# hwb0314/VI-ORB-SLAM-ICRA2018

Hardware: AMD Instinct MI355X
Metric: ORB extract+match frames/sec @640x480/1000 feat (higher is better)
Workload: dtype u8

## Files before the change

vi-orb-slam-icra2018_amd/csrc/k_pyramid.hip:

```cpp
#include "orbhip_internal.h"
#include "wave_ops.h"

#include <algorithm>

#define RZ_TW 128
typedef unsigned short us2 __attribute__((ext_vector_type(2)));
#define RZ_MAXCH 16
#define RZ_MAXROWS 44

template <int RZ_TH>
__global__ __launch_bounds__(256) void k_resize(const uint8_t *__restrict__ src, int sstride,
                                                unsigned long long sframe, uint8_t *__restrict__ dst,
                                                int dw, int dh, int dstride, unsigned long long dframe,
                                                const int2 *__restrict__ xtab,
                                                const int4 *__restrict__ ytab, const int4 *__restrict__ gtab, int sw, int sh,
                                                float winx, float winy, int xcdMap)
{
    __shared__ __align__(16) uint8_t s_src[RZ_MAXROWS + 1][RZ_MAXCH * 16];
    const int tid = threadIdx.x;
    const int tilesX = (dw + RZ_TW - 1) / RZ_TW, tilesY = (dh + RZ_TH - 1) / RZ_TH;
    const int t = xcd_tile(xcdMap), frame = blockIdx.y;
    if (t >= tilesX * tilesY) return;
    const int by = t / tilesX, bx = t - by * tilesX;
    const int ox0 = bx * RZ_TW, oy0 = by * RZ_TH;
// ... 163 lines not shown
    const int ox1 = min(ox0 + (twg << 2), dw) - 1, oy1 = min(oy0 + TH, dh) - 1;
    const uint8_t *S = src + (size_t)frame * sframe;
    uint8_t *D = dst + (size_t)frame * dframe;
    const int sxmin = max((int)((float)ox0 * winx) - 1, 0), sxmax = min((int)((float)(ox1 + 1) * winx) + 1, sw - 1);
    const int symin = max((int)((float)oy0 * winy) - 1, 0), symax = min((int)((float)(oy1 + 1) * winy) + 1, sh - 1);
    const int XA = sxmin & ~15;
    const int nch = ((sxmax - XA) >> 4) + 1, nrows = symax - symin + 1;
    {
        const int lane = tid & 63, wv = __builtin_amdgcn_readfirstlane(tid >> 6);
        const int rl = lane >> 4, ch = lane & 15;
        const uint8_t *sp = S + (size_t)(symin + rl) * sstride + XA + (ch << 4);
        const uint32_t ldsBase = (uint32_t)(uintptr_t)&s_src[0][0];
        for (int rb = wv * 4; rb < nrows; rb += 16)
            if (ch < nch && rb + rl < nrows) glds16(sp + (size_t)rb * sstride, ldsBase + (uint32_t)(rb * (RZ_MAXCH * 16)));
        if (wv == 1) {
            if (lane < TH) glds16(ytab + min(oy0 + lane, dh - 1), (uint32_t)(uintptr_t)&s_ytab[0]);
        } else if (wv >= 2) {
            const int q = 64 * (wv - 2) + lane;
            const int grp = q / 3, part = q - 3 * grp;
            if (q < 3 * twg) glds16(gtab + 3 * (min(ox0 + 4 * grp, dw - 1) >> 2) + part, (uint32_t)(uintptr_t)&s_gtab[64 * (wv - 2)]);
        }
    }
    const int r = (int)(((unsigned)tid * (unsigned)rmagic) >> 16), g = tid - r * twg;
    const int gx = ox0 + (g << 2);
    const bool live = r < rpp && gx < dw;
    asm volatile("s_waitcnt vmcnt(0)" ::: "memory");
    __syncthreads();
    if (!live) return;
    const int4 *gp = s_gtab + 3 * g;
    const int4 g0 = gp[0], gsel = gp[1], gw = gp[2];
    const int bcol = g0.x - XA, wb = bcol & ~3, shf = bcol & 3;
    const uint32_t sel[4] = {(uint32_t)gsel.x, (uint32_t)gsel.y, (uint32_t)gsel.z, (uint32_t)gsel.w};
    const uint32_t wt[4] = {(uint32_t)gw.x, (uint32_t)gw.y, (uint32_t)gw.z, (uint32_t)gw.w};
    for (int j = 0; j < npass; j++) {
        const int ry = r + rpp * j, dy = oy0 + ry;
        if (dy >= dh) break;
        const int4 ytj = s_ytab[ry];
        const uint32_t b0s = ((uint32_t)ytj.z & 0xFFFu) << 12, b1s = ((uint32_t)ytj.w & 0xFFFu) << 12;
        const uint32_t *q0 = reinterpret_cast<const uint32_t *>(&s_src[ytj.x - symin][wb]);
        const uint32_t *q1 = reinterpret_cast<const uint32_t *>(&s_src[ytj.y - symin][wb]);
        const uint32_t a0 = q0[0], a1 = q0[1], a2 = q0[2], c0 = q1[0], c1 = q1[1], c2 = q1[2];
        const uint32_t lo0 = __builtin_amdgcn_alignbyte(a1, a0, shf), hi0 = __builtin_amdgcn_alignbyte(a2, a1, shf);
        const uint32_t lo1 = __builtin_amdgcn_alignbyte(c1, c0, shf), hi1 = __builtin_amdgcn_alignbyte(c2, c1, shf);
        uint32_t v[4];
#pragma unroll
        for (int k = 0; k < 4; k++) {
            const us2 p0 = __builtin_bit_cast(us2, __builtin_amdgcn_perm(hi0, lo0, sel[k]));
            const us2 p1 = __builtin_bit_cast(us2, __builtin_amdgcn_perm(hi1, lo1, sel[k]));
            const us2 w2 = __builtin_bit_cast(us2, wt[k]);
            const uint32_t r0 = __builtin_amdgcn_udot2(p0, w2, 0u, false);
            const uint32_t r1 = __builtin_amdgcn_udot2(p1, w2, 0u, false);
            v[k] = (__umulhi(b0s, r0 & 0x7FFFF0u) + __umulhi(b1s, r1 & 0x7FFFF0u) + 2u) >> 2;
        }
        const uint32_t packed = v[0] | (v[1] << 8) | (v[2] << 16) | (v[3] << 24);
        uint8_t *o = D + (size_t)dy * dstride + gx;
        if (gx + 3 < dw) {
            *reinterpret_cast<uint32_t *>(o) = packed;
        } else {
            for (int k = 0; k < 4 && gx + k < dw; k++) o[k] = (uint8_t)(packed >> (8 * k));
        }
    }
}

bool resize_fit_plan(const int32_t *xt, const int32_t *yt, int sw, int sh, int dw, int dh, ResizeFit &out)
{
    const int ng = (dw + 3) / 4;
    const float winx = (float)sw / (float)dw, winy = (float)sh / (float)dh;
    long best = -1;
    for (int ntx = (ng + 31) / 32; ntx <= (ng + 31) / 32 + 3; ntx++) {
        const int twg = (ng + ntx - 1) / ntx;
        if (twg < 8 || twg > 32) continue;
        const int rpp = 256 / twg, rmagic = (65536 + twg - 1) / twg;
        bool okMagic = true;
        for (int tid = 0; tid < 256; tid++) okMagic = okMagic && (int)(((unsigned)tid * (unsigned)rmagic) >> 16) == tid / twg;
        if (!okMagic) continue;
        for (int npass = 3; npass <= 6; npass++) {
            const int TH = rpp * npass;
            if (TH > RF_MAXTH) continue;
            const int nty = (dh + TH - 1) / TH;
            const long cost = (long)ntx * nty * (100 + 70 * npass);
            if (best >= 0 && cost >= best) continue;
            bool ok = true;
            for (int bx = 0; bx < ntx && ok; bx++) {
                const int ox0 = bx * 4 * twg, ox1 = std::min(ox0 + 4 * twg, dw) - 1;
                if (ox0 >= dw) { ok = false; break; }
                const int lo = std::max((int)((float)ox0 * winx) - 1, 0), hi = std::min((int)((float)(ox1 + 1) * winx) + 1, sw - 1);
                if (lo > (xt[2 * ox0] & 0xFFFF) || hi < (int)((uint32_t)xt[2 * ox1] >> 16)) ok = false;
                if (((hi - (lo & ~15)) >> 4) + 1 > RZ_MAXCH) ok = false;
            }
            for (int by = 0; by < nty && ok; by++) {
                const int oy0 = by * TH, oy1 = std::min(oy0 + TH, dh) - 1;
                const int rlo = std::max((int)((float)oy0 * winy) - 1, 0), rhi = std::min((int)((float)(oy1 + 1) * winy) + 1, sh - 1);
                if (rlo > yt[4 * oy0] || rhi < yt[4 * oy1 + 1] || rhi - rlo + 1 > RF_MAXROWS) ok = false;
            }
            if (!ok) continue;
            best = cost;
            out.ntx = ntx; out.nty = nty; out.twg = twg; out.rpp = rpp; out.npass = npass; out.rmagic = rmagic;
        }
    }
    return best >= 0;
}

void launch_resize_fit(hipStream_t s, const uint8_t *src, int sw, int sh, int sstride, size_t sframe, uint8_t *dst, int dw, int dh,
                       int dstride, size_t dframe, const int32_t *ytab, const int32_t *gtab, const ResizeFit &f, int B)
{
    dim3 grid(orb_xcd_pad(f.ntx * f.nty), B, 1), block(256, 1, 1);
    orb_path(ORB_PATH_RESIZE_FIT);
    hipLaunchKernelGGL(k_resize_fit, grid, block, 0, s, src, sstride, (unsigned long long)sframe, dst, dw, dh, dstride,
                       (unsigned long long)dframe, reinterpret_cast<const int4 *>(ytab), reinterpret_cast<const int4 *>(gtab), sw, sh,
                       (float)sw / (float)dw, (float)sh / (float)dh, 1, f.ntx, f.nty, f.twg, f.rpp, f.npass, f.rmagic);
}

static bool resize_window_hint_ok(const int32_t *xt, const int32_t *yt, int sw, int sh, int dw, int dh, int th, float winx,
                                  float winy)
{
    for (int ox0 = 0; ox0 < dw; ox0 += RZ_TW) {
        const int ox1 = std::min(ox0 + RZ_TW, dw) - 1;
        const int lo = std::max((int)((float)ox0 * winx) - 1, 0), hi = std::min((int)((float)(ox1 + 1) * winx) + 1, sw - 1);
        if (lo > (xt[2 * ox0] & 0xFFFF) || hi < (int)((uint32_t)xt[2 * ox1] >> 16)) return false;
        const int nch = ((hi - (lo & ~15)) >> 4) + 1;
        if (nch > RZ_MAXCH) return false;
        for (int oy0 = 0; oy0 < dh; oy0 += th) {
            const int oy1 = std::min(oy0 + th, dh) - 1;
            const int rlo = std::max((int)((float)oy0 * winy) - 1, 0), rhi = std::min((int)((float)(oy1 + 1) * winy) + 1, sh - 1);
            if (rlo > yt[4 * oy0] || rhi < yt[4 * oy1 + 1]) return false;
            const int nrows = rhi - rlo + 1;
            if (nrows > RZ_MAXROWS || nrows * nch > 512) return false;
        }
    }
    return true;
}
// ... 292 lines not shown
```

vi-orb-slam-icra2018_amd/csrc/k_bowseq.hip:

```cpp
#include "orbhip_internal.h"
#include "wave_ops.h"

#include <type_traits>

#include <cstdlib>

#define BS_HISTO 30

#define BS_THREADS 1024

struct BsBest {
    int b1, pos, b2;
};

__device__ __forceinline__ int bs_bound(const unsigned long long *keys, int n, unsigned node, bool upper)
{
    int lo = 0, hi = n;
    while (lo < hi) {
        const int mid = (lo + hi) >> 1;
        const unsigned v = (unsigned)(keys[mid] >> 32);
        if (upper ? (v <= node) : (v < node))
            lo = mid + 1;
        else
            hi = mid;
    }
    return lo;
}

__device__ void bs_sort2(unsigned long long *keysA, unsigned long long *keysB, int NP, int tid)
{
    auto exchange = [&](int t, int k, int j) {
        unsigned long long *keys = t < NP / 2 ? keysA : keysB;
        const int u = t < NP / 2 ? t : t - NP / 2;
        const int i = ((u & ~(j - 1)) << 1) | (u & (j - 1));
// ... 377 lines not shown
            }
            s_keep[0] = i1;
            s_keep[1] = i2;
            s_keep[2] = i3;
        }
        __syncthreads();
    }
    (void)mybin0;
    for (int i = tid; i < cap; i += blockDim.x) o21[i] = -1;
    __syncthreads();
    int local = 0;
    for (int i1 = tid; i1 < cap; i1 += blockDim.x) {
        int i2 = i1 < n1 ? m12[i1] : -1;
        if (i2 >= 0 && check_ori) {
            float rot = k1[i1].angle - k2[i2].angle;
            if (rot < 0.0f) rot += 360.0f;
            int bin = (int)roundf(rot * (1.0f / BS_HISTO));
            if (bin == BS_HISTO) bin = 0;
            if (bin >= 0 && bin < BS_HISTO && bin != s_keep[0] && bin != s_keep[1] && bin != s_keep[2]) i2 = -1;
        }
        o12[i1] = i2;
        if (i2 >= 0) {
            o21[i2] = i1;
            local++;
        }
    }
    atomicAdd(&s_nm, local);
    __syncthreads();
    if (tid == 0) nmatches[b] = s_nm;
}


#define BL_THREADS 512
#define BL_TILES 640
#define BL_MAXN2 128

__device__ __forceinline__ int bl_dist(const uint4 &q0, const uint4 &q1, const uint4 &r0, const uint4 &r1)
{
    return __popc(q0.x ^ r0.x) + __popc(q0.y ^ r0.y) + __popc(q0.z ^ r0.z) + __popc(q0.w ^ r0.w) + __popc(q1.x ^ r1.x) +
           __popc(q1.y ^ r1.y) + __popc(q1.z ^ r1.z) + __popc(q1.w ^ r1.w);
}

__global__ __launch_bounds__(BL_THREADS, 3) void k_bow_lane(const uint8_t *__restrict__ desc, const orbhip_keypoint *__restrict__ kps,
                                                        const int32_t *__restrict__ counts, const int32_t *__restrict__ node,
                                                        const float *__restrict__ weight, const uint8_t *__restrict__ valid, int cap,
                                                        int NP, int lag, int th, int th_mode, float nnratio, int check_ori,
                                                        int32_t *__restrict__ match12, int32_t *__restrict__ match21,
                                                        int32_t *__restrict__ nmatches ORB_ABL_PARAM)
{
    extern __shared__ __align__(16) uint8_t smem[];
    const int capP = (cap + 63) & ~63;
    unsigned long long *key1 = reinterpret_cast<unsigned long long *>(smem);
    unsigned long long *key2 = key1 + NP;
    uint8_t *dist = smem;
    const int dcap = NP * 16 - BL_TILES * 4;
    uint32_t *tiles = reinterpret_cast<uint32_t *>(smem + dcap);
    uint16_t *idx1 = reinterpret_cast<uint16_t *>(smem + (size_t)NP * 16);
    uint16_t *idx2 = idx1 + capP;
    uint16_t *m12 = idx2 + capP;
    uint2 *items = reinterpret_cast<uint2 *>(m12 + capP);
    uint16_t *ioff = reinterpret_cast<uint16_t *>(items + capP);
    uint16_t *order = ioff + capP;
    unsigned *claim = reinterpret_cast<unsigned *>(order + capP);
    unsigned *vbit1 = claim + NP / 32, *vbit2 = vbit1 + NP / 32;
    __shared__ int s_n1v, s_n2v, s_nitems, s_next, s_nm, s_over, s_ntiles;
    __shared__ int s_cls[4], s_cur[4];
    __shared__ int s_hist[BS_HISTO];
    __shared__ int s_keep[3];

    const int b = blockIdx.x;
    const int tid = threadIdx.x, lane = tid & 63;
    const int n2 = min(counts[b], cap);
    int32_t *o12 = match12 + (size_t)b * cap;
    int32_t *o21 = match21 + (size_t)b * cap;
    if (b < lag) {
        for (int i = tid; i < cap; i += BL_THREADS) {
            o12[i] = -1;
            o21[i] = -1;
        }
        if (tid == 0) nmatches[b] = 0;
        return;
    }
    const int b1 = b - lag;
    const int n1 = min(counts[b1], cap);
    const uint8_t *d1 = desc + (size_t)b1 * cap * 32, *d2 = desc + (size_t)b * cap * 32;
    const int32_t *nd1 = node + (size_t)b1 * cap, *nd2 = node + (size_t)b * cap;
    const float *w1 = weight + (size_t)b1 * cap, *w2 = weight + (size_t)b * cap;
    int NS = 64;
    while (NS < max(n1, n2)) NS <<= 1;

    for (int i = tid; i < NS; i += BL_THREADS) {
        key1[i] = (i < n1 && w1[i] > 0.f) ? (((unsigned long long)(unsigned)nd1[i] << 32) | (unsigned)i) : ~0ull;
        key2[i] = (i < n2 && w2[i] > 0.f) ? (((unsigned long long)(unsigned)nd2[i] << 32) | (unsigned)i) : ~0ull;
    }
    for (int i = tid; i < capP; i += BL_THREADS) m12[i] = 0xFFFFu;
    for (int i = tid; i < NP / 32; i += BL_THREADS) {
        claim[i] = 0;
        unsigned v1 = 0xFFFFFFFFu, v2 = 0xFFFFFFFFu;
        if (valid) {
            v1 = v2 = 0;
            for (int k = 0; k < 32; k++) {
                const int f = i * 32 + k;
                if (f < n1 && valid[(size_t)b1 * cap + f]) v1 |= 1u << k;
                if (f < n2 && valid[(size_t)b * cap + f]) v2 |= 1u << k;
            }
        }
        vbit1[i] = v1;
        vbit2[i] = v2;
    }
    if (tid < BS_HISTO) s_hist[tid] = 0;
    if (tid == 0) {
        s_n1v = 0;
        s_n2v = 0;
        s_nitems = 0;
        s_cls[0] = s_cls[1] = s_cls[2] = s_cls[3] = 0;
        s_cur[0] = s_cur[1] = s_cur[2] = s_cur[3] = 0;
        s_next = 0;
        s_nm = 0;
        s_over = 0;
        s_ntiles = 0;
    }
    __syncthreads();
    ORB_ABL_STOP(phases < 1);
    bs_sort2(key1, key2, NS, tid);
    ORB_ABL_STOP(phases < 2);
    for (int i = tid; i < NS; i += BL_THREADS) {
        if (key1[i] != ~0ull && (i + 1 == NS || key1[i + 1] == ~0ull)) s_n1v = i + 1;
        if (key2[i] != ~0ull && (i + 1 == NS || key2[i + 1] == ~0ull)) s_n2v = i + 1;
    }
    __syncthreads();
    const int n1v = s_n1v, n2v = s_n2v;

    for (int p = tid; p < n1v; p += BL_THREADS) {
        idx1[p] = (uint16_t)(unsigned)key1[p];
        const unsigned nodeId = (unsigned)(key1[p] >> 32);
        if (p == 0 || (unsigned)(key1[p - 1] >> 32) != nodeId) {
            const int s2 = bs_bound(key2, n2v, nodeId, false), e2 = bs_bound(key2, n2v, nodeId, true);
            if (e2 > s2) {
                const int e1 = bs_bound(key1, n1v, nodeId, true);
                const int slot = atomicAdd(&s_nitems, 1);
                items[slot] = make_uint2((unsigned)p | ((unsigned)e1 << 16), (unsigned)s2 | ((unsigned)e2 << 16));
            }
        }
    }
    for (int p = tid; p < n2v; p += BL_THREADS) idx2[p] = (uint16_t)(unsigned)key2[p];
    __syncthreads();
    ORB_ABL_STOP(phases < 3);
    const int nitems = s_nitems;

    auto class_of = [&](const uint2 it) {
        const int c2 = (int)((it.y >> 16) - (it.y & 0xFFFF));
        return c2 > BL_MAXN2 ? 3 : c2 > 64 ? 0 : c2 > 16 ? 1 : 2;
    };
    for (int i = tid; i < nitems; i += BL_THREADS) atomicAdd(&s_cls[class_of(items[i])], 1);
    __syncthreads();
    const int ngroup8 = s_cls[0], ngroup = ngroup8 + s_cls[1], nmat = ngroup + s_cls[2];
    for (int i = tid; i < nitems; i += BL_THREADS) {
        const int cls = class_of(items[i]);
        const int r = (cls == 0 ? 0 : cls == 1 ? ngroup8 : cls == 2 ? ngroup : nmat) + atomicAdd(&s_cur[cls], 1);
        order[r] = (uint16_t)i;
    }
    __syncthreads();
    if (tid < 64) {
        int base = 0, tbase = 0;
        for (int r0 = 0; r0 < nmat; r0 += 64) {
            const int r = r0 + lane;
            int units = 0;
            if (r < nmat) {
                const uint2 it = items[order[r]];
                units = (int)((it.x >> 16) - (it.x & 0xFFFF)) * (int)((((it.y >> 16) - (it.y & 0xFFFF)) + 3) >> 2);
            }
            int incl = units;
#pragma unroll
            for (int d = 1; d < 64; d <<= 1) {
                const int o = __shfl_up(incl, d);
                if (lane >= d) incl += o;
            }
            const int start = base + incl - units;
            int ntl = 0, tR = 0, tC = 0;
            if (r < nmat) {
                const uint2 it = items[order[r]];
                tR = ((int)((it.x >> 16) - (it.x & 0xFFFF)) + 15) >> 4;
                tC = ((int)((it.y >> 16) - (it.y & 0xFFFF)) + 15) >> 4;
                ntl = tR * tC;
            }
            int tincl = ntl;
#pragma unroll
            for (int d = 1; d < 64; d <<= 1) {
                const int o = __shfl_up(tincl, d);
                if (lane >= d) tincl += o;
            }
            const int tstart = tbase + tincl - ntl;
            const bool fits = (start + units) * 4 <= dcap && start + units < 0xFFFF && tR <= 16 && tstart + ntl <= BL_TILES;
            if (r < nmat) ioff[order[r]] = fits ? (uint16_t)start : (uint16_t)0xFFFFu;
            if (r < nmat)
                for (int k = 0; k < ntl && tstart + k < BL_TILES; k++)
                    tiles[tstart + k] = fits ? ((uint32_t)r | ((uint32_t)(k / tC) << 11) | ((uint32_t)(k % tC) << 15)) : 0xFFFFFFFFu;
            if (__ballot(r < nmat && !fits) && lane == 0) s_over = 1;
            base += __shfl(incl, 63);
            tbase += __shfl(tincl, 63);
        }
        if (lane == 0) s_ntiles = min(tbase, BL_TILES);
    }
    for (int r = nmat + tid; r < nitems; r += BL_THREADS) ioff[order[r]] = 0xFFFFu;
    __syncthreads();
    ORB_ABL_STOP(phases < 4);
    const int ntiles = s_ntiles;

    {
        const int gl = lane & 15, grp = tid >> 4, ngrp = BL_THREADS >> 4;
        const uint4 *D1 = reinterpret_cast<const uint4 *>(d1), *D2 = reinterpret_cast<const uint4 *>(d2);
        struct Tile {
            int off, stride, nrow, c, row0;
            bool hasC;
        };
        uint4 q0, q1, r0, r1, nq0, nq1, nr0, nr1;
        Tile T, NT;
        auto fetch = [&](int t, Tile &X, uint4 &a0, uint4 &a1, uint4 &b0, uint4 &b1) {
            const uint32_t e0 = tiles[t];
            const bool empty = e0 == 0xFFFFFFFFu;
            const uint32_t e = empty ? 0u : e0;
            const int slot = order[e & 0x7FF], tr = (e >> 11) & 15, tc = (e >> 15) & 15;
            const uint2 it = items[slot];
            const int s1 = it.x & 0xFFFF, n1i = (int)(it.x >> 16) - s1, s2 = it.y & 0xFFFF, n2i = (int)(it.y >> 16) - s2;
            X.off = ioff[slot];
            X.stride = (n2i + 3) & ~3;
            X.nrow = empty || X.off == 0xFFFF ? 0 : n1i;
            X.row0 = tr * 16;
            X.c = tc * 16 + gl;
            X.hasC = X.c < n2i;
            const int i1 = idx1[s1 + min(tr * 16 + gl, n1i - 1)];
            const int i2 = idx2[s2 + min(X.c, n2i - 1)];
            a0 = D1[2 * i1];
            a1 = D1[2 * i1 + 1];
            b0 = D2[2 * i2];
            b1 = D2[2 * i2 + 1];
        };
        int t = grp;
        if (t < ntiles) fetch(t, NT, nq0, nq1, nr0, nr1);
        for (; t < ntiles; t += ngrp) {
            T = NT;
            q0 = nq0; q1 = nq1; r0 = nr0; r1 = nr1;
            if (t + ngrp < ntiles) fetch(t + ngrp, NT, nq0, nq1, nr0, nr1);
            uint8_t *dst = dist + (size_t)T.off * 4 + T.c;
            const bool inPad = T.c < T.stride;
#define BL_STEP(U)                                                                                                              \
    {                                                                                                                           \
        const int row = T.row0 + ((gl - (U)) & 15);                                                                            \
        uint32_t x0, x1, x2, x3, x4, x5, x6, x7;                                                                                \
        if ((U) == 0) {                                                                                                         \
            x0 = q0.x ^ r0.x; x1 = q0.y ^ r0.y; x2 = q0.z ^ r0.z; x3 = q0.w ^ r0.w;                                             \
            x4 = q1.x ^ r1.x; x5 = q1.y ^ r1.y; x6 = q1.z ^ r1.z; x7 = q1.w ^ r1.w;                                             \
        } else                                                                                                                  \
            asm volatile("s_nop 1\n\t"                                                                                          \
                         "v_xor_b32_dpp %0, %8, %16 row_ror:" #U " row_mask:0xf bank_mask:0xf\n\t"                              \
                         "v_xor_b32_dpp %1, %9, %17 row_ror:" #U " row_mask:0xf bank_mask:0xf\n\t"                              \
                         "v_xor_b32_dpp %2, %10, %18 row_ror:" #U " row_mask:0xf bank_mask:0xf\n\t"                             \
                         "v_xor_b32_dpp %3, %11, %19 row_ror:" #U " row_mask:0xf bank_mask:0xf\n\t"                             \
                         "v_xor_b32_dpp %4, %12, %20 row_ror:" #U " row_mask:0xf bank_mask:0xf\n\t"                             \
                         "v_xor_b32_dpp %5, %13, %21 row_ror:" #U " row_mask:0xf bank_mask:0xf\n\t"                             \
                         "v_xor_b32_dpp %6, %14, %22 row_ror:" #U " row_mask:0xf bank_mask:0xf\n\t"                             \
                         "v_xor_b32_dpp %7, %15, %23 row_ror:" #U " row_mask:0xf bank_mask:0xf"                                 \
                         : "=&v"(x0), "=&v"(x1), "=&v"(x2), "=&v"(x3), "=&v"(x4), "=&v"(x5), "=&v"(x6), "=&v"(x7)               \
                         : "v"(q0.x), "v"(q0.y), "v"(q0.z), "v"(q0.w), "v"(q1.x), "v"(q1.y), "v"(q1.z), "v"(q1.w), "v"(r0.x),   \
                           "v"(r0.y), "v"(r0.z), "v"(r0.w), "v"(r1.x), "v"(r1.y), "v"(r1.z), "v"(r1.w));                        \
        const int d = __popc(x0) + __popc(x1) + __popc(x2) + __popc(x3) + __popc(x4) + __popc(x5) + __popc(x6) + __popc(x7);    \
        if (inPad && row < T.nrow) dst[(size_t)row * T.stride] = (uint8_t)(T.hasC ? min(d, 255) : 255);                         \
    }
            BL_STEP(0) BL_STEP(1) BL_STEP(2) BL_STEP(3) BL_STEP(4) BL_STEP(5) BL_STEP(6) BL_STEP(7)
            BL_STEP(8) BL_STEP(9) BL_STEP(10) BL_STEP(11) BL_STEP(12) BL_STEP(13) BL_STEP(14) BL_STEP(15)
#undef BL_STEP
        }
    }
    __syncthreads();
    ORB_ABL_STOP(phases < 5);

    {
        const int gl = lane & 15, grp = tid >> 4, ngrp = BL_THREADS >> 4;
        auto group_item = [&](auto jtag, int r) {
            constexpr int J = decltype(jtag)::value;
            const int slot = order[r];
            const int off = ioff[slot];
            if (off == 0xFFFF) return;
            const uint2 it = items[slot];
            const int s1 = it.x & 0xFFFF, nrow = (int)(it.x >> 16) - s1, s2 = it.y & 0xFFFF, n2i = (int)(it.y >> 16) - s2;
            const int stride = (n2i + 3) & ~3;
            uint32_t gm[J];
#pragma unroll
            for (int j = 0; j < J; j++) {
                const int c = gl + 16 * j;
                bool out = c >= n2i;
                if (!out && th_mode) {
                    const int i2 = idx2[s2 + c];
                    out = !((vbit2[i2 >> 5] >> (i2 & 31)) & 1u);
                }
                gm[j] = out ? 0xFFu : 0u;
            }
            const uint8_t *rowp = dist + (size_t)off * 4 + gl;
            const uint32_t *idx1w = reinterpret_cast<const uint32_t *>(idx1);
            const bool checkValid = valid != nullptr;
            uint32_t dn[J], iwn;
#pragma unroll
            for (int j = 0; j < J; j++) dn[j] = rowp[16 * j];
            iwn = idx1w[s1 >> 1];
            for (int a = 0; a < nrow; a++) {
                const int i1 = (int)((iwn >> (16 * ((s1 + a) & 1))) & 0xFFFFu);
                uint32_t dj[J];
#pragma unroll
                for (int j = 0; j < J; j++) dj[j] = dn[j] | gm[j];
                rowp += stride;
                if (a + 1 < nrow) {
#pragma unroll
                    for (int j = 0; j < J; j++) dn[j] = rowp[16 * j];
                    iwn = idx1w[(s1 + a + 1) >> 1];
                }
                if (checkValid && !((vbit1[i1 >> 5] >> (i1 & 31)) & 1u)) continue;
                unsigned k1 = 0xFFFFFFu, k2 = (256u << 8);
#pragma unroll
                for (int j = 0; j < J; j++) {
                    const unsigned key = (dj[j] << 8) | (unsigned)(gl + 16 * j);
                    unsigned nk2;
                    asm("v_med3_u32 %0, %1, %2, %3" : "=v"(nk2) : "v"(k1), "v"(k2), "v"(key));
                    k1 = min(k1, key);
                    k2 = nk2;
                }
                const int K1 = row_min((int)k1);
                const int K2 = row_min((int)(k1 == (unsigned)K1 ? k2 : k1));
                const int bd1 = K1 >> 8, bd2 = K2 >> 8, pos = K1 & 0xFF;
                const bool pass = th_mode ? (bd1 < th) : (bd1 <= th);
                if (pass && (float)bd1 < nnratio * (float)bd2) {
                    if ((pos & 15) == gl) {
#pragma unroll
                        for (int j = 0; j < J; j++)
                            if ((pos >> 4) == j) gm[j] = 0xFFu;
                        m12[i1] = idx2[s2 + pos];
                    }
                }
            }
        };
        const int g8pad = (ngroup8 + 3) & ~3, n4 = ngroup - ngroup8;
        for (int g = grp; g < g8pad + n4; g += ngrp) {
            if (g < ngroup8)
                group_item(std::integral_constant<int, 8>{}, g);
            else if (g >= g8pad)
                group_item(std::integral_constant<int, 4>{}, ngroup8 + (g - g8pad));
        }
    }
    for (int r = ngroup + (BL_THREADS - 1 - tid); r < nmat; r += BL_THREADS) {
        const int slot = order[r];
        const int off = ioff[slot];
        if (off == 0xFFFF) continue;
        const uint2 it = items[slot];
        const int s1 = it.x & 0xFFFF, nrow = (int)(it.x >> 16) - s1, s2 = it.y & 0xFFFF, n2i = (int)(it.y >> 16) - s2;
        const int nw = (n2i + 3) >> 2;
        uint32_t cm[4] = {0u, 0u, 0u, 0u};
        if (th_mode) {
            for (int c = 0; c < n2i; c++) {
                const int i2 = idx2[s2 + c];
                if (!((vbit2[i2 >> 5] >> (i2 & 31)) & 1u)) {
                    const uint32_t m = 0xFFu << (8 * (c & 3));
#pragma unroll
                    for (int k = 0; k < 4; k++)
                        if ((c >> 2) == k) cm[k] |= m;
                }
            }
        }
        const uint32_t *row = reinterpret_cast<const uint32_t *>(dist + (size_t)off * 4);
        const uint32_t *idx1w = reinterpret_cast<const uint32_t *>(idx1);
        const bool checkValid = valid != nullptr;
        const uint32_t padm[4] = {0u, nw > 1 ? 0u : 0xFFFFFFFFu, nw > 2 ? 0u : 0xFFFFFFFFu, nw > 3 ? 0u : 0xFFFFFFFFu};
        uint32_t wn[4], iwn;
#pragma unroll
        for (int k = 0; k < 4; k++) wn[k] = row[k];
        iwn = idx1w[s1 >> 1];
        for (int a = 0; a < nrow; a++) {
            const int i1 = (int)((iwn >> (16 * ((s1 + a) & 1))) & 0xFFFFu);
            uint32_t w[4];
#pragma unroll
            for (int k = 0; k < 4; k++) w[k] = wn[k] | cm[k] | padm[k];
            row += nw;
            if (a + 1 < nrow) {
#pragma unroll
                for (int k = 0; k < 4; k++) wn[k] = row[k];
                iwn = idx1w[(s1 + a + 1) >> 1];
            }
// ... 5 lines not shown
#pragma unroll
                    for (int q = 0; q < 4; q++) {
                        const unsigned key = (((w[k] >> (8 * q)) & 0xFFu) << 8) | (unsigned)(4 * k + q);
                        unsigned nk2;
                        asm("v_med3_u32 %0, %1, %2, %3" : "=v"(nk2) : "v"(k1), "v"(k2), "v"(key));
                        k1 = min(k1, key);
                        k2 = nk2;
                    }
                }
            }
            const int bd1 = (int)(k1 >> 8), bd2 = (int)(k2 >> 8), pos = (int)(k1 & 0xFFu);
            const bool pass = th_mode ? (bd1 < th) : (bd1 <= th);
            if (pass && (float)bd1 < nnratio * (float)bd2) {
                m12[i1] = idx2[s2 + pos];
                const uint32_t m = 0xFFu << (8 * (pos & 3));
#pragma unroll
                for (int k = 0; k < 4; k++)
                    if ((pos >> 2) == k) cm[k] |= m;
            }
        }
    }
    __syncthreads();
    ORB_ABL_STOP(phases < 6);

    const int firstCoop = s_over ? 0 : nmat;
    if (firstCoop >= nitems) goto rotation;
    if (tid == 0) s_next = firstCoop;
    __syncthreads();
    for (;;) {
        int rr = 0;
        if (lane == 0) rr = atomicAdd(&s_next, 1);
        rr = __builtin_amdgcn_readfirstlane(rr);
        if (rr >= nitems) break;
        const int slot = order[rr];
        if (ioff[slot] != 0xFFFF) continue;
        const uint2 it = items[slot];
        const int e1 = it.x >> 16, s2 = it.y & 0xFFFF, e2 = it.y >> 16;
        for (int a = it.x & 0xFFFF; a < e1; a++) {
            const int i1 = __builtin_amdgcn_readfirstlane((int)idx1[a]);
            if (!((vbit1[i1 >> 5] >> (i1 & 31)) & 1u)) continue;
            const uint4 q0 = reinterpret_cast<const uint4 *>(d1)[2 * i1], q1 = reinterpret_cast<const uint4 *>(d1)[2 * i1 + 1];
            BsBest B = {256, 0x7FFFFFFF, 256};
            for (int p = s2 + lane; p < e2; p += 64) {
                const int i2 = idx2[p];
                if ((claim[i2 >> 5] >> (i2 & 31)) & 1u) continue;
                if (th_mode && !((vbit2[i2 >> 5] >> (i2 & 31)) & 1u)) continue;
                const uint4 r0 = reinterpret_cast<const uint4 *>(d2)[2 * i2], r1 = reinterpret_cast<const uint4 *>(d2)[2 * i2 + 1];
                const int d = bl_dist(q0, q1, r0, r1);
                if (d < B.b1) {
                    B.b2 = B.b1;
                    B.b1 = d;
                    B.pos = p;
                } else if (d < B.b2) {
                    B.b2 = d;
                }
            }
            const int key = B.b1 < 256 ? ((B.b1 << 16) | B.pos) : 0x7FFFFFFF;
            const int k1 = wave_min(key);
            const int k2 = wave_min(key == k1 ? B.b2 : B.b1);
            const int bd1 = k1 == 0x7FFFFFFF ? 256 : (k1 >> 16), bd2 = k2;
            const bool pass = th_mode ? (bd1 < th) : (bd1 <= th);
            if (pass && (float)bd1 < nnratio * (float)bd2) {
                const int i2 = idx2[k1 & 0xFFFF];
                if (lane == 0) {
                    m12[i1] = (uint16_t)i2;
                    atomicOr(&claim[i2 >> 5], 1u << (i2 & 31));
                }
                __builtin_amdgcn_fence(__ATOMIC_RELEASE, "wavefront");
                __builtin_amdgcn_wave_barrier();
// ... 51 lines not shown
    }
    for (int i = tid; i < cap; i += BL_THREADS) o21[i] = -1;
    __syncthreads();
    int local = 0;
    for (int i1 = tid; i1 < cap; i1 += BL_THREADS) {
        int i2 = i1 < n1 ? (int)m12[i1] : 0xFFFF;
        if (i2 == 0xFFFF) i2 = -1;
        if (i2 >= 0 && check_ori) {
            const int bin = bin_of(i1, i2);
            if (bin >= 0 && bin < BS_HISTO && bin != s_keep[0] && bin != s_keep[1] && bin != s_keep[2]) i2 = -1;
        }
        o12[i1] = i2;
        if (i2 >= 0) {
            o21[i2] = i1;
            local++;
        }
    }
    atomicAdd(&s_nm, local);
    __syncthreads();
    if (tid == 0) nmatches[b] = s_nm;
}

hipError_t launch_bow_seq(hipStream_t s, const uint8_t *desc, const orbhip_keypoint *kps, const int32_t *counts,
                          const int32_t *node, const float *weight, const uint8_t *valid, int cap, int B, int lag, int th,
                          int th_mode, float nnratio, int check_ori, int32_t *match12, int32_t *match21,
                          int32_t *nmatches)
{
    if (B <= 0) return hipSuccess;
    int NP = 512;
    while (NP < cap) NP <<= 1;
    static const int laneEnv = ORB_TUNE("BOW_LANE", 1);
    {
        const int capP = (cap + 63) & ~63;
        const size_t ldsLane = (size_t)NP * 16 + (size_t)capP * (3 * 2 + 8 + 2 + 2) + (size_t)NP / 32 * 12 + 64;
        if (laneEnv && cap < 65535 && NP <= 4096 && ldsLane <= 150 * 1024 && (float)th < nnratio * 255.0f && th < 255) {
            static const int dbgL = ORB_TUNE("BOW_PHASES", 9);
            (void)dbgL;
            hipError_t e = hipSuccess;
            if (ldsLane > 48 * 1024) e = hipFuncSetAttribute((const void *)k_bow_lane, hipFuncAttributeMaxDynamicSharedMemorySize, (int)ldsLane);
            if (e == hipSuccess) {
                (void)hipGetLastError();
                hipLaunchKernelGGL(k_bow_lane, dim3(B, 1, 1), dim3(BL_THREADS, 1, 1), ldsLane, s, desc, kps, counts, node, weight, valid, cap,
                                   NP, lag, th, th_mode, nnratio, check_ori, match12, match21, nmatches ORB_ABL_ARG(dbgL));
                e = hipGetLastError();
            }
            if (e == hipSuccess) {
                orb_path(ORB_PATH_BOW_LANE);
                return hipSuccess;
            }
            (void)hipGetLastError();
        }
    }
    const size_t base = (((size_t)NP * 36 + (size_t)NP / 32 * 12 + 15) & ~(size_t)15) + 64;
    const size_t full = base + (size_t)cap * 64;
    static const int forceGlobal = ORB_TUNE("BOW_GLOBAL_DESC", 0);
    const bool ldsd = full <= 150 * 1024 && !forceGlobal;
    static const int dbg = ORB_TUNE("BOW_PHASES", 9);
    (void)dbg;
    const size_t lds = ldsd ? full : base;
    const void *fn = ldsd ? (const void *)k_bow_seq<true> : (const void *)k_bow_seq<false>;
    if (lds > 48 * 1024) {
        const hipError_t e = hipFuncSetAttribute(fn, hipFuncAttributeMaxDynamicSharedMemorySize, (int)lds);
        if (e != hipSuccess) return e;
    }
    orb_path(ldsd ? ORB_PATH_BOW_SEQ_LDS : ORB_PATH_BOW_SEQ_GLOBAL);
    if (ldsd)
        hipLaunchKernelGGL(k_bow_seq<true>, dim3(B, 1, 1), dim3(BS_THREADS, 1, 1), lds, s, desc, kps, counts, node, weight, valid,
                           cap, NP, lag, th, th_mode, nnratio, check_ori, match12, match21, nmatches ORB_ABL_ARG(dbg));
    else
        hipLaunchKernelGGL(k_bow_seq<false>, dim3(B, 1, 1), dim3(BS_THREADS, 1, 1), lds, s, desc, kps, counts, node, weight, valid,
                           cap, NP, lag, th, th_mode, nnratio, check_ori, match12, match21, nmatches ORB_ABL_ARG(dbg));
    return hipGetLastError();
}
```

Before: 363,200.

## Assign consecutive rows per thread in resize-fit and reuse horizontal filter results

```diff
diff --git a/vi-orb-slam-icra2018_amd/csrc/k_pyramid.hip b/vi-orb-slam-icra2018_amd/csrc/k_pyramid.hip
--- a/vi-orb-slam-icra2018_amd/csrc/k_pyramid.hip
+++ b/vi-orb-slam-icra2018_amd/csrc/k_pyramid.hip
@@ -219,34 +219,78 @@
     const int bcol = g0.x - XA, wb = bcol & ~3, shf = bcol & 3;
     const uint32_t sel[4] = {(uint32_t)gsel.x, (uint32_t)gsel.y, (uint32_t)gsel.z, (uint32_t)gsel.w};
     const uint32_t wt[4] = {(uint32_t)gw.x, (uint32_t)gw.y, (uint32_t)gw.z, (uint32_t)gw.w};
-    for (int j = 0; j < npass; j++) {
-        const int ry = r + rpp * j, dy = oy0 + ry;
-        if (dy >= dh) break;
-        const int4 ytj = s_ytab[ry];
+    const int ry0 = r * npass, dyFirst = oy0 + ry0;
+    const int nrun = min(npass, dh - dyFirst);
+    const uint8_t *ldsRow = &s_src[0][0];
+    const int rowOff = wb - symin * (RZ_MAXCH * 16);
+    auto form = [&](int y, uint32_t (&Hs)[4]) {
+        const uint32_t *q = reinterpret_cast<const uint32_t *>(ldsRow + (rowOff + y * (RZ_MAXCH * 16)));
+        const uint32_t a0 = q[0], a1 = q[1], a2 = q[2];
+        const uint32_t lo = __builtin_amdgcn_alignbyte(a1, a0, shf), hi = __builtin_amdgcn_alignbyte(a2, a1, shf);
+#pragma unroll
+        for (int k = 0; k < 4; k++) {
+            const us2 p = __builtin_bit_cast(us2, __builtin_amdgcn_perm(hi, lo, sel[k]));
+            Hs[k] = __builtin_amdgcn_udot2(p, __builtin_bit_cast(us2, wt[k]), 0u, false) & 0x7FFFF0u;
+        }
+    };
+    const int4 *yp = s_ytab + ry0;
+    uint32_t off = (uint32_t)dyFirst * (uint32_t)dstride + (uint32_t)gx;
+    const bool whole = gx + 3 < dw;
+    int prevY1 = -1;
+    auto row = [&](const int4 ytj, uint32_t (&H0)[4], uint32_t (&H1)[4]) {
+        if (ytj.x != prevY1) form(ytj.x, H0);
+        form(ytj.y, H1);
+        prevY1 = ytj.y;
         const uint32_t b0s = ((uint32_t)ytj.z & 0xFFFu) << 12, b1s = ((uint32_t)ytj.w & 0xFFFu) << 12;
-        const uint32_t *q0 = reinterpret_cast<const uint32_t *>(&s_src[ytj.x - symin][wb]);
-        const uint32_t *q1 = reinterpret_cast<const uint32_t *>(&s_src[ytj.y - symin][wb]);
-        const uint32_t a0 = q0[0], a1 = q0[1], a2 = q0[2], c0 = q1[0], c1 = q1[1], c2 = q1[2];
-        const uint32_t lo0 = __builtin_amdgcn_alignbyte(a1, a0, shf), hi0 = __builtin_amdgcn_alignbyte(a2, a1, shf);
-        const uint32_t lo1 = __builtin_amdgcn_alignbyte(c1, c0, shf), hi1 = __builtin_amdgcn_alignbyte(c2, c1, shf);
         uint32_t v[4];
 #pragma unroll
         for (int k = 0; k < 4; k++) {
-            const us2 p0 = __builtin_bit_cast(us2, __builtin_amdgcn_perm(hi0, lo0, sel[k]));
-            const us2 p1 = __builtin_bit_cast(us2, __builtin_amdgcn_perm(hi1, lo1, sel[k]));
-            const us2 w2 = __builtin_bit_cast(us2, wt[k]);
-            const uint32_t r0 = __builtin_amdgcn_udot2(p0, w2, 0u, false);
-            const uint32_t r1 = __builtin_amdgcn_udot2(p1, w2, 0u, false);
-            v[k] = (__umulhi(b0s, r0 & 0x7FFFF0u) + __umulhi(b1s, r1 & 0x7FFFF0u) + 2u) >> 2;
+            __builtin_assume(H0[k] < (1u << 24));
+            v[k] = (__umulhi(b0s, H0[k]) + __umulhi(b1s, H1[k]) + 2u) >> 2;
         }
         const uint32_t packed = v[0] | (v[1] << 8) | (v[2] << 16) | (v[3] << 24);
-        uint8_t *o = D + (size_t)dy * dstride + gx;
-        if (gx + 3 < dw) {
+        uint8_t *o = D + off;
+        if (whole) {
             *reinterpret_cast<uint32_t *>(o) = packed;
         } else {
             for (int k = 0; k < 4 && gx + k < dw; k++) o[k] = (uint8_t)(packed >> (8 * k));
         }
-    }
+        off += (uint32_t)dstride;
+    };
+    uint32_t P[4] = {0u, 0u, 0u, 0u}, Q[4] = {0u, 0u, 0u, 0u};
+    int j = 0;
+    for (; j + 1 < nrun; j += 2, yp += 2) {
+        const int4 ya = yp[0], yb = yp[1];
+        row(ya, P, Q);
+        row(yb, Q, P);
+    }
+    if (j < nrun) row(yp[0], P, Q);
+}
+
+#define RF_I_FIXED 100
+#define RF_I_ROW 64
+#define RF_I_FORM 21
+
+static long resize_fit_cost(const int32_t *yt, int dh, int twg, int rpp, int npass)
+{
+    const int TH = rpp * npass, nty = (dh + TH - 1) / TH;
+    long cost = 0;
+    for (int by = 0; by < nty; by++)
+        for (int w = 0; w < 4; w++) {
+            cost += RF_I_FIXED;
+            const int r0 = (64 * w) / twg, r1 = std::min((64 * w + 63) / twg, rpp - 1);
+            for (int j = 0; j < npass; j++) {
+                bool any = false, form = false;
+                for (int r = r0; r <= r1; r++) {
+                    const int dy = by * TH + r * npass + j;
+                    if (dy >= dh) continue;
+                    any = true;
+                    form = form || j == 0 || yt[4 * dy] != yt[4 * (dy - 1) + 1];
+                }
+                if (any) cost += RF_I_ROW + (form ? RF_I_FORM : 0);
+            }
+        }
+    return cost;
 }
 
 bool resize_fit_plan(const int32_t *xt, const int32_t *yt, int sw, int sh, int dw, int dh, ResizeFit &out)
@@ -257,33 +301,33 @@
     for (int ntx = (ng + 31) / 32; ntx <= (ng + 31) / 32 + 3; ntx++) {
         const int twg = (ng + ntx - 1) / ntx;
         if (twg < 8 || twg > 32) continue;
-        const int rpp = 256 / twg, rmagic = (65536 + twg - 1) / twg;
+        const int rmagic = (65536 + twg - 1) / twg;
         bool okMagic = true;
         for (int tid = 0; tid < 256; tid++) okMagic = okMagic && (int)(((unsigned)tid * (unsigned)rmagic) >> 16) == tid / twg;
         if (!okMagic) continue;
-        for (int npass = 3; npass <= 6; npass++) {
-            const int TH = rpp * npass;
-            if (TH > RF_MAXTH) continue;
-            const int nty = (dh + TH - 1) / TH;
-            const long cost = (long)ntx * nty * (100 + 70 * npass);
-            if (best >= 0 && cost >= best) continue;
-            bool ok = true;
-            for (int bx = 0; bx < ntx && ok; bx++) {
-                const int ox0 = bx * 4 * twg, ox1 = std::min(ox0 + 4 * twg, dw) - 1;
-                if (ox0 >= dw) { ok = false; break; }
-                const int lo = std::max((int)((float)ox0 * winx) - 1, 0), hi = std::min((int)((float)(ox1 + 1) * winx) + 1, sw - 1);
-                if (lo > (xt[2 * ox0] & 0xFFFF) || hi < (int)((uint32_t)xt[2 * ox1] >> 16)) ok = false;
-                if (((hi - (lo & ~15)) >> 4) + 1 > RZ_MAXCH) ok = false;
+        for (int rpp = 256 / twg; rpp * twg > 192; rpp--)
+            for (int npass = 3; rpp * npass <= RF_MAXTH; npass++) {
+                const int TH = rpp * npass;
+                const int nty = (dh + TH - 1) / TH;
+                const long cost = (long)ntx * resize_fit_cost(yt, dh, twg, rpp, npass);
+                if (best >= 0 && cost >= best) continue;
+                bool ok = true;
+                for (int bx = 0; bx < ntx && ok; bx++) {
+                    const int ox0 = bx * 4 * twg, ox1 = std::min(ox0 + 4 * twg, dw) - 1;
+                    if (ox0 >= dw) { ok = false; break; }
+                    const int lo = std::max((int)((float)ox0 * winx) - 1, 0), hi = std::min((int)((float)(ox1 + 1) * winx) + 1, sw - 1);
+                    if (lo > (xt[2 * ox0] & 0xFFFF) || hi < (int)((uint32_t)xt[2 * ox1] >> 16)) ok = false;
+                    if (((hi - (lo & ~15)) >> 4) + 1 > RZ_MAXCH) ok = false;
+                }
+                for (int by = 0; by < nty && ok; by++) {
+                    const int oy0 = by * TH, oy1 = std::min(oy0 + TH, dh) - 1;
+                    const int rlo = std::max((int)((float)oy0 * winy) - 1, 0), rhi = std::min((int)((float)(oy1 + 1) * winy) + 1, sh - 1);
+                    if (rlo > yt[4 * oy0] || rhi < yt[4 * oy1 + 1] || rhi - rlo + 1 > RF_MAXROWS) ok = false;
+                }
+                if (!ok) continue;
+                best = cost;
+                out.ntx = ntx; out.nty = nty; out.twg = twg; out.rpp = rpp; out.npass = npass; out.rmagic = rmagic;
             }
-            for (int by = 0; by < nty && ok; by++) {
-                const int oy0 = by * TH, oy1 = std::min(oy0 + TH, dh) - 1;
-                const int rlo = std::max((int)((float)oy0 * winy) - 1, 0), rhi = std::min((int)((float)(oy1 + 1) * winy) + 1, sh - 1);
-                if (rlo > yt[4 * oy0] || rhi < yt[4 * oy1 + 1] || rhi - rlo + 1 > RF_MAXROWS) ok = false;
-            }
-            if (!ok) continue;
-            best = cost;
-            out.ntx = ntx; out.nty = nty; out.twg = twg; out.rpp = rpp; out.npass = npass; out.rmagic = rmagic;
-        }
     }
     return best >= 0;
 }
```

Measured after the change: 364,900 (median of 6 runs). About the same (+0.5%).

## Compact BoW lane kernel LDS arena and raise occupancy target

Applied to the files above, without the earlier changes.

```diff
diff --git a/vi-orb-slam-icra2018_amd/csrc/bow_sort_core.h b/vi-orb-slam-icra2018_amd/csrc/bow_sort_core.h
--- /dev/null
+++ b/vi-orb-slam-icra2018_amd/csrc/bow_sort_core.h
@@ -0,0 +1,87 @@
+#ifndef ORBHIP_BOW_SORT_CORE_H
+#define ORBHIP_BOW_SORT_CORE_H
+
+#if defined(__HIPCC__)
+#define BSC_HD __host__ __device__ __forceinline__
+#else
+#define BSC_HD inline
+#endif
+
+BSC_HD void bow_sort_cx(unsigned long long &lo, unsigned long long &hi)
+{
+    const unsigned long long a = lo, b = hi;
+    lo = a < b ? a : b;
+    hi = a < b ? b : a;
+}
+
+BSC_HD void bow_sort_quad(unsigned long long *keysA, unsigned long long *keysB, int L, int NS, int t, int k, int j)
+{
+    unsigned long long *keys = t < NS / 4 ? keysA : keysB;
+    const int v = t < NS / 4 ? t : t - NS / 4, h = j >> 1;
+    const bool mirrored = j == (k >> 1);
+    const int p0 = ((v & ~(h - 1)) << 2) | (v & (h - 1)), p1 = p0 + h;
+    const int p3 = mirrored ? (p0 ^ (k - 1)) : p1 + j, p2 = p3 - h;
+    if (p1 >= L) return;
+    unsigned long long a0 = keys[p0], a1 = keys[p1], a2 = p2 < L ? keys[p2] : ~0ull, a3 = p3 < L ? keys[p3] : ~0ull;
+    if (mirrored) {
+        bow_sort_cx(a0, a3);
+        bow_sort_cx(a1, a2);
+    } else {
+        bow_sort_cx(a0, a2);
+        bow_sort_cx(a1, a3);
+    }
+    bow_sort_cx(a0, a1);
+    bow_sort_cx(a2, a3);
+    keys[p0] = a0;
+    keys[p1] = a1;
+    if (p2 < L) keys[p2] = a2;
+    if (p3 < L) keys[p3] = a3;
+}
+
+BSC_HD void bow_sort_pairs(unsigned long long *keysA, unsigned long long *keysB, int L, int NS, int t)
+{
+    unsigned long long *keys = t < NS / 4 ? keysA : keysB;
+    const int p = 4 * (t < NS / 4 ? t : t - NS / 4);
+    if (p + 1 < L) {
+        unsigned long long a = keys[p], b = keys[p + 1];
+        bow_sort_cx(a, b);
+        keys[p] = a;
+        keys[p + 1] = b;
+    }
+    if (p + 3 < L) {
+        unsigned long long a = keys[p + 2], b = keys[p + 3];
+        bow_sort_cx(a, b);
+        keys[p + 2] = a;
+        keys[p + 3] = b;
+    }
+}
+
+template <class X>
+BSC_HD void bow_sort2(X &x, unsigned long long *keysA, unsigned long long *keysB, int L, int NS)
+{
+    for (int k = 2; k <= NS; k <<= 1) {
+        for (int j = k >> 1; j > 0;) {
+            for (int t = x.first(); t < NS / 2; t += x.stride()) {
+                if (j >= 2)
+                    bow_sort_quad(keysA, keysB, L, NS, t, k, j);
+                else
+                    bow_sort_pairs(keysA, keysB, L, NS, t);
+            }
+            const bool crossed = j > 32;
+            j >>= j >= 2 ? 2 : 1;
+            if (crossed || (j > 0 ? j : k) > 32)
+                x.sync();
+            else
+                x.wave_sync();
+        }
+    }
+}
+
+struct BowSortSerial {
+    int first() const { return 0; }
+    int stride() const { return 1; }
+    void sync() const {}
+    void wave_sync() const {}
+};
+
+#endif
diff --git a/vi-orb-slam-icra2018_amd/csrc/k_bowseq.hip b/vi-orb-slam-icra2018_amd/csrc/k_bowseq.hip
--- a/vi-orb-slam-icra2018_amd/csrc/k_bowseq.hip
+++ b/vi-orb-slam-icra2018_amd/csrc/k_bowseq.hip
@@ -1,5 +1,6 @@
 #include "orbhip_internal.h"
 #include "wave_ops.h"
+#include "bow_sort_core.h"
 
 #include <type_traits>
 
@@ -443,6 +444,7 @@
 
 
 #define BL_THREADS 512
+#define BL_WAVES_PER_SIMD 8
 #define BL_TILES 640
 #define BL_MAXN2 128
 
@@ -452,28 +454,50 @@
            __popc(q1.y ^ r1.y) + __popc(q1.z ^ r1.z) + __popc(q1.w ^ r1.w);
 }
 
-__global__ __launch_bounds__(BL_THREADS, 3) void k_bow_lane(const uint8_t *__restrict__ desc, const orbhip_keypoint *__restrict__ kps,
+struct BlItem {
+    uint32_t x, y;
+    uint16_t ioff;
+    uint16_t order;
+};
+
+static inline __host__ __device__ int bl_arena(int capP)
+{
+    const int a = capP * (2 * 8 + (int)sizeof(BlItem));
+    return a < 8192 ? 8192 : a;
+}
+
+struct BlBlock {
+    int tid;
+    __device__ int first() const { return tid; }
+    __device__ int stride() const { return BL_THREADS; }
+    __device__ void sync() const { __syncthreads(); }
+    __device__ void wave_sync() const
+    {
+        __builtin_amdgcn_fence(__ATOMIC_RELEASE, "wavefront");
+        __builtin_amdgcn_wave_barrier();
+        __builtin_amdgcn_fence(__ATOMIC_ACQUIRE, "wavefront");
+    }
+};
+
+__global__ __launch_bounds__(BL_THREADS, BL_WAVES_PER_SIMD) void k_bow_lane(const uint8_t *__restrict__ desc, const orbhip_keypoint *__restrict__ kps,
                                                         const int32_t *__restrict__ counts, const int32_t *__restrict__ node,
                                                         const float *__restrict__ weight, const uint8_t *__restrict__ valid, int cap,
-                                                        int NP, int lag, int th, int th_mode, float nnratio, int check_ori,
+                                                        int lag, int th, int th_mode, float nnratio, int check_ori,
                                                         int32_t *__restrict__ match12, int32_t *__restrict__ match21,
                                                         int32_t *__restrict__ nmatches ORB_ABL_PARAM)
 {
     extern __shared__ __align__(16) uint8_t smem[];
-    const int capP = (cap + 63) & ~63;
+    const int capP = (cap + 63) & ~63, arena = bl_arena(capP);
     unsigned long long *key1 = reinterpret_cast<unsigned long long *>(smem);
-    unsigned long long *key2 = key1 + NP;
+    unsigned long long *key2 = key1 + capP;
     uint8_t *dist = smem;
-    const int dcap = NP * 16 - BL_TILES * 4;
-    uint32_t *tiles = reinterpret_cast<uint32_t *>(smem + dcap);
-    uint16_t *idx1 = reinterpret_cast<uint16_t *>(smem + (size_t)NP * 16);
+    BlItem *const top = reinterpret_cast<BlItem *>(smem + arena);
+    uint16_t *idx1 = reinterpret_cast<uint16_t *>(smem + arena);
     uint16_t *idx2 = idx1 + capP;
     uint16_t *m12 = idx2 + capP;
-    uint2 *items = reinterpret_cast<uint2 *>(m12 + capP);
-    uint16_t *ioff = reinterpret_cast<uint16_t *>(items + capP);
-    uint16_t *order = ioff + capP;
-    unsigned *claim = reinterpret_cast<unsigned *>(order + capP);
-    unsigned *vbit1 = claim + NP / 32, *vbit2 = vbit1 + NP / 32;
+    unsigned *claim = reinterpret_cast<unsigned *>(m12 + capP);
+    unsigned *vbit1 = claim + capP / 32, *vbit2 = vbit1 + capP / 32;
+    auto item_of = [&](int slot) { return make_uint2(top[-1 - slot].x, top[-1 - slot].y); };
     __shared__ int s_n1v, s_n2v, s_nitems, s_next, s_nm, s_over, s_ntiles;
     __shared__ int s_cls[4], s_cur[4];
     __shared__ int s_hist[BS_HISTO];
@@ -499,13 +523,14 @@
     const float *w1 = weight + (size_t)b1 * cap, *w2 = weight + (size_t)b * cap;
     int NS = 64;
     while (NS < max(n1, n2)) NS <<= 1;
-
-    for (int i = tid; i < NS; i += BL_THREADS) {
+    const int L = min(NS, capP);
+
+    for (int i = tid; i < L; i += BL_THREADS) {
         key1[i] = (i < n1 && w1[i] > 0.f) ? (((unsigned long long)(unsigned)nd1[i] << 32) | (unsigned)i) : ~0ull;
         key2[i] = (i < n2 && w2[i] > 0.f) ? (((unsigned long long)(unsigned)nd2[i] << 32) | (unsigned)i) : ~0ull;
     }
     for (int i = tid; i < capP; i += BL_THREADS) m12[i] = 0xFFFFu;
-    for (int i = tid; i < NP / 32; i += BL_THREADS) {
+    for (int i = tid; i < capP / 32; i += BL_THREADS) {
         claim[i] = 0;
         unsigned v1 = 0xFFFFFFFFu, v2 = 0xFFFFFFFFu;
         if (valid) {
@@ -533,11 +558,14 @@
     }
     __syncthreads();
     ORB_ABL_STOP(phases < 1);
-    bs_sort2(key1, key2, NS, tid);
+    {
+        BlBlock x = {tid};
+        bow_sort2(x, key1, key2, L, NS);
+    }
     ORB_ABL_STOP(phases < 2);
-    for (int i = tid; i < NS; i += BL_THREADS) {
-        if (key1[i] != ~0ull && (i + 1 == NS || key1[i + 1] == ~0ull)) s_n1v = i + 1;
-        if (key2[i] != ~0ull && (i + 1 == NS || key2[i + 1] == ~0ull)) s_n2v = i + 1;
+    for (int i = tid; i < L; i += BL_THREADS) {
+        if (key1[i] != ~0ull && (i + 1 == L || key1[i + 1] == ~0ull)) s_n1v = i + 1;
+        if (key2[i] != ~0ull && (i + 1 == L || key2[i + 1] == ~0ull)) s_n2v = i + 1;
     }
     __syncthreads();
     const int n1v = s_n1v, n2v = s_n2v;
@@ -550,7 +578,8 @@
             if (e2 > s2) {
                 const int e1 = bs_bound(key1, n1v, nodeId, true);
                 const int slot = atomicAdd(&s_nitems, 1);
-                items[slot] = make_uint2((unsigned)p | ((unsigned)e1 << 16), (unsigned)s2 | ((unsigned)e2 << 16));
+                top[-1 - slot].x = (unsigned)p | ((unsigned)e1 << 16);
+                top[-1 - slot].y = (unsigned)s2 | ((unsigned)e2 << 16);
             }
         }
     }
@@ -558,18 +587,20 @@
     __syncthreads();
     ORB_ABL_STOP(phases < 3);
     const int nitems = s_nitems;
+    uint32_t *tiles = reinterpret_cast<uint32_t *>(top - nitems) - BL_TILES;
+    const int dcap = (int)(reinterpret_cast<uint8_t *>(tiles) - smem);
 
     auto class_of = [&](const uint2 it) {
         const int c2 = (int)((it.y >> 16) - (it.y & 0xFFFF));
         return c2 > BL_MAXN2 ? 3 : c2 > 64 ? 0 : c2 > 16 ? 1 : 2;
     };
-    for (int i = tid; i < nitems; i += BL_THREADS) atomicAdd(&s_cls[class_of(items[i])], 1);
+    for (int i = tid; i < nitems; i += BL_THREADS) atomicAdd(&s_cls[class_of(item_of(i))], 1);
     __syncthreads();
     const int ngroup8 = s_cls[0], ngroup = ngroup8 + s_cls[1], nmat = ngroup + s_cls[2];
     for (int i = tid; i < nitems; i += BL_THREADS) {
-        const int cls = class_of(items[i]);
+        const int cls = class_of(item_of(i));
         const int r = (cls == 0 ? 0 : cls == 1 ? ngroup8 : cls == 2 ? ngroup : nmat) + atomicAdd(&s_cur[cls], 1);
-        order[r] = (uint16_t)i;
+        top[-1 - r].order = (uint16_t)i;
     }
     __syncthreads();
     if (tid < 64) {
@@ -578,7 +609,7 @@
             const int r = r0 + lane;
             int units = 0;
             if (r < nmat) {
-                const uint2 it = items[order[r]];
+                const uint2 it = item_of(top[-1 - r].order);
                 units = (int)((it.x >> 16) - (it.x & 0xFFFF)) * (int)((((it.y >> 16) - (it.y & 0xFFFF)) + 3) >> 2);
             }
             int incl = units;
@@ -590,7 +621,7 @@
             const int start = base + incl - units;
             int ntl = 0, tR = 0, tC = 0;
             if (r < nmat) {
-                const uint2 it = items[order[r]];
+                const uint2 it = item_of(top[-1 - r].order);
                 tR = ((int)((it.x >> 16) - (it.x & 0xFFFF)) + 15) >> 4;
                 tC = ((int)((it.y >> 16) - (it.y & 0xFFFF)) + 15) >> 4;
                 ntl = tR * tC;
@@ -603,7 +634,7 @@
             }
             const int tstart = tbase + tincl - ntl;
             const bool fits = (start + units) * 4 <= dcap && start + units < 0xFFFF && tR <= 16 && tstart + ntl <= BL_TILES;
-            if (r < nmat) ioff[order[r]] = fits ? (uint16_t)start : (uint16_t)0xFFFFu;
+            if (r < nmat) top[-1 - top[-1 - r].order].ioff = fits ? (uint16_t)start : (uint16_t)0xFFFFu;
             if (r < nmat)
                 for (int k = 0; k < ntl && tstart + k < BL_TILES; k++)
                     tiles[tstart + k] = fits ? ((uint32_t)r | ((uint32_t)(k / tC) << 11) | ((uint32_t)(k % tC) << 15)) : 0xFFFFFFFFu;
@@ -613,7 +644,7 @@
         }
         if (lane == 0) s_ntiles = min(tbase, BL_TILES);
     }
-    for (int r = nmat + tid; r < nitems; r += BL_THREADS) ioff[order[r]] = 0xFFFFu;
+    for (int r = nmat + tid; r < nitems; r += BL_THREADS) top[-1 - top[-1 - r].order].ioff = 0xFFFFu;
     __syncthreads();
     ORB_ABL_STOP(phases < 4);
     const int ntiles = s_ntiles;
@@ -625,16 +656,16 @@
             int off, stride, nrow, c, row0;
             bool hasC;
         };
-        uint4 q0, q1, r0, r1, nq0, nq1, nr0, nr1;
-        Tile T, NT;
+        uint4 q0, q1, r0, r1;
+        Tile T;
         auto fetch = [&](int t, Tile &X, uint4 &a0, uint4 &a1, uint4 &b0, uint4 &b1) {
             const uint32_t e0 = tiles[t];
             const bool empty = e0 == 0xFFFFFFFFu;
             const uint32_t e = empty ? 0u : e0;
-            const int slot = order[e & 0x7FF], tr = (e >> 11) & 15, tc = (e >> 15) & 15;
-            const uint2 it = items[slot];
+            const int slot = top[-1 - (int)(e & 0x7FF)].order, tr = (e >> 11) & 15, tc = (e >> 15) & 15;
+            const uint2 it = item_of(slot);
             const int s1 = it.x & 0xFFFF, n1i = (int)(it.x >> 16) - s1, s2 = it.y & 0xFFFF, n2i = (int)(it.y >> 16) - s2;
-            X.off = ioff[slot];
+            X.off = top[-1 - slot].ioff;
             X.stride = (n2i + 3) & ~3;
             X.nrow = empty || X.off == 0xFFFF ? 0 : n1i;
             X.row0 = tr * 16;
@@ -647,12 +678,8 @@
             b0 = D2[2 * i2];
             b1 = D2[2 * i2 + 1];
         };
-        int t = grp;
-        if (t < ntiles) fetch(t, NT, nq0, nq1, nr0, nr1);
-        for (; t < ntiles; t += ngrp) {
-            T = NT;
-            q0 = nq0; q1 = nq1; r0 = nr0; r1 = nr1;
-            if (t + ngrp < ntiles) fetch(t + ngrp, NT, nq0, nq1, nr0, nr1);
+        for (int t = grp; t < ntiles; t += ngrp) {
+            fetch(t, T, q0, q1, r0, r1);
             uint8_t *dst = dist + (size_t)T.off * 4 + T.c;
             const bool inPad = T.c < T.stride;
 #define BL_STEP(U)                                                                                                              \
@@ -690,10 +717,10 @@
         const int gl = lane & 15, grp = tid >> 4, ngrp = BL_THREADS >> 4;
         auto group_item = [&](auto jtag, int r) {
             constexpr int J = decltype(jtag)::value;
-            const int slot = order[r];
-            const int off = ioff[slot];
+            const int slot = top[-1 - r].order;
+            const int off = top[-1 - slot].ioff;
             if (off == 0xFFFF) return;
-            const uint2 it = items[slot];
+            const uint2 it = item_of(slot);
             const int s1 = it.x & 0xFFFF, nrow = (int)(it.x >> 16) - s1, s2 = it.y & 0xFFFF, n2i = (int)(it.y >> 16) - s2;
             const int stride = (n2i + 3) & ~3;
             uint32_t gm[J];
@@ -758,10 +785,10 @@
         }
     }
     for (int r = ngroup + (BL_THREADS - 1 - tid); r < nmat; r += BL_THREADS) {
-        const int slot = order[r];
-        const int off = ioff[slot];
+        const int slot = top[-1 - r].order;
+        const int off = top[-1 - slot].ioff;
         if (off == 0xFFFF) continue;
-        const uint2 it = items[slot];
+        const uint2 it = item_of(slot);
         const int s1 = it.x & 0xFFFF, nrow = (int)(it.x >> 16) - s1, s2 = it.y & 0xFFFF, n2i = (int)(it.y >> 16) - s2;
         const int nw = (n2i + 3) >> 2;
         uint32_t cm[4] = {0u, 0u, 0u, 0u};
@@ -833,9 +860,9 @@
         if (lane == 0) rr = atomicAdd(&s_next, 1);
         rr = __builtin_amdgcn_readfirstlane(rr);
         if (rr >= nitems) break;
-        const int slot = order[rr];
-        if (ioff[slot] != 0xFFFF) continue;
-        const uint2 it = items[slot];
+        const int slot = top[-1 - rr].order;
+        if (top[-1 - slot].ioff != 0xFFFF) continue;
+        const uint2 it = item_of(slot);
         const int e1 = it.x >> 16, s2 = it.y & 0xFFFF, e2 = it.y >> 16;
         for (int a = it.x & 0xFFFF; a < e1; a++) {
             const int i1 = __builtin_amdgcn_readfirstlane((int)idx1[a]);
@@ -953,7 +980,7 @@
     static const int laneEnv = ORB_TUNE("BOW_LANE", 1);
     {
         const int capP = (cap + 63) & ~63;
-        const size_t ldsLane = (size_t)NP * 16 + (size_t)capP * (3 * 2 + 8 + 2 + 2) + (size_t)NP / 32 * 12 + 64;
+        const size_t ldsLane = (size_t)bl_arena(capP) + (size_t)capP * 3 * 2 + (size_t)capP / 32 * 12;
         if (laneEnv && cap < 65535 && NP <= 4096 && ldsLane <= 150 * 1024 && (float)th < nnratio * 255.0f && th < 255) {
             static const int dbgL = ORB_TUNE("BOW_PHASES", 9);
             (void)dbgL;
@@ -962,7 +989,7 @@
             if (e == hipSuccess) {
                 (void)hipGetLastError();
                 hipLaunchKernelGGL(k_bow_lane, dim3(B, 1, 1), dim3(BL_THREADS, 1, 1), ldsLane, s, desc, kps, counts, node, weight, valid, cap,
-                                   NP, lag, th, th_mode, nnratio, check_ori, match12, match21, nmatches ORB_ABL_ARG(dbgL));
+                                   lag, th, th_mode, nnratio, check_ori, match12, match21, nmatches ORB_ABL_ARG(dbgL));
                 e = hipGetLastError();
             }
             if (e == hipSuccess) {
```

New measurement: 362,700 before, 365,400 after, median of 4. No clear change (+0.7%).
